# docknetwork/crypto

Measured on AMD Instinct MI355X. Metric: BLS12-381 G1 MSM/s at n=2^20 (1 GPU) and n=2^24 (8 GPU); bit-exact vs CPU, higher is better.
Workload: dtype i32 (13 signed 30-bit limbs, 381-bit modular integer; 64-bit column accumulators)

## Files before the change

crypto_amd/csrc/dock_ctx.hpp:

```cpp
#pragma once
#include <hip/hip_runtime.h>
#include <algorithm>
#include <atomic>
#include <condition_variable>
#include <cstdlib>
#include <cstring>
#include <map>
#include <mutex>
#include <vector>
#include "../../include/dock_gpu.h"
#include "host_par.hpp"

namespace dock {

extern std::atomic<uint64_t> g_dev_allocs, g_dev_alloc_ns, g_dev_alloc_bytes;
hipError_t dev_malloc(void **p, size_t bytes);

struct Buf {
    void *p = nullptr; size_t cap = 0;
    int32_t ensure(size_t bytes) {
        if (bytes <= cap) return DGPU_OK;
        if (p) { (void)hipFree(p); p = nullptr; cap = 0; }
        size_t want = bytes + bytes / 8 + 256;
        if (dev_malloc(&p, want) != hipSuccess) { (void)hipGetLastError(); if (dev_malloc(&p, bytes) != hipSuccess) { p = nullptr; return DGPU_E_OOM; } want = bytes; }
        cap = want; return DGPU_OK;
    }
    void release() { if (p) (void)hipFree(p); p = nullptr; cap = 0; }
    template <class T> T *as() { return reinterpret_cast<T *>(p); }
};

struct Handle { void *p; size_t n; int kind; int ctx; int inflight; void *aux = nullptr; int small_uses = 0; };
struct PreTable { void *tab; size_t n; int c, W; };
struct SortedScalars { void *off, *entries; size_t off_bytes, entries_bytes; size_t n, rows, boff; int c, W; };
struct FoldTab { void *tab; size_t bytes; size_t n; };
struct ShardSet { std::vector<uint64_t> sub; std::vector<size_t> lo; size_t n = 0; };
struct NttDomain { void *tw_f = nullptr, *tw_i = nullptr, *pw_f = nullptr, *pw_i = nullptr, *zinv = nullptr, *pwr_f = nullptr, *pwr_i = nullptr; };

struct ProfEntry { const char *name; double ms; uint64_t calls; };

struct Shared;
extern Shared gs;
#define HIPCHK(x) do { hipError_t e_ = (x); if (e_ != hipSuccess) { dock::gs.last_hip = (int32_t)e_; (void)hipGetLastError(); return DGPU_E_HIP; } } while (0)

struct Slot {
    std::mutex mu;
    hipStream_t stream = nullptr;
    static constexpr int N_COPY_EV = 15;
    hipStream_t cstream = nullptr;
    hipStream_t xstream = nullptr;
    void *hpin = nullptr;
    static constexpr size_t HPIN_BYTES = 64 * 1024;
    void *hpin2 = nullptr; size_t hpin2_bytes = 0;
    hipEvent_t copy_ev[N_COPY_EV + 1] = {};
    unsigned ev_next = 0;
    Buf flags, in_bases, in_inf, in_scalars, prepped, digits, heavy, cnt, off, cursor, bsums, entries, bucket, bucket_inf, head, tail, head_b, tail_b, part_inf, l1, l1_inf, win, win_inf, ml_lines, ml_partial, ml_out, ml_coeffs, ml_state, dyn, hpart, hpart_inf, small_cnt;
    Buf q[16];
    std::vector<std::pair<const char *, std::pair<hipEvent_t, hipEvent_t>>> prof_pending;
    std::vector<hipEvent_t> ev_pool;
    void release_all() {
        Buf *bufs[] = {&flags, &in_bases, &in_inf, &in_scalars, &prepped, &digits, &heavy, &cnt, &off, &cursor, &bsums, &entries, &bucket, &bucket_inf, &head, &tail, &head_b, &tail_b, &part_inf, &l1, &l1_inf, &win, &win_inf, &ml_lines, &ml_partial, &ml_out, &ml_coeffs, &ml_state, &dyn, &hpart, &hpart_inf, &small_cnt};
        for (Buf *b : bufs) b->release();
        for (Buf &b : q) b.release();
        for (hipEvent_t e : ev_pool) (void)hipEventDestroy(e);
        ev_pool.clear(); prof_pending.clear();
    }
};
constexpr int N_SLOTS = 6;

constexpr int MAX_CTX = 16;
struct Ctx {
    std::atomic<bool> ready{false};
    int device = -1;
    Slot slots[N_SLOTS];
    std::atomic<unsigned> rr{0};
    std::mutex slot_mu; std::condition_variable slot_cv; uint64_t slot_next = 0, slot_serving = 0; bool slot_taken[N_SLOTS] = {};
    std::atomic<int> busy{0};
    std::atomic<int> ml_active{0};
    std::map<int, NttDomain> ntt_domains;
    std::vector<std::pair<void *, size_t>> scalar_pool;
    size_t scalar_pool_bytes = 0;
    std::vector<std::pair<void *, size_t>> fold_pool;
};
constexpr size_t SCALAR_POOL_MAX_ENTRIES = 32, SCALAR_POOL_MAX_BYTES = (size_t)4 << 30;
struct Shared {
    std::mutex mu;
    std::mutex small_mu;
    std::condition_variable cv;
    std::map<uint64_t, Handle> handles;
    uint64_t next_handle = 1;
    std::atomic<int32_t> last_hip{0};
    std::atomic<size_t> min_gpu_n{DGPU_DEFAULT_MIN_GPU_N};
    std::atomic<size_t> auto_shard_min_n{~(size_t)0};
    std::atomic<int> window_bits{0};
// ... 146 lines not shown
```

crypto_amd/csrc/dock_dev.hip:

```cpp
#include "msm_driver.hip.h"
#include "../../include/dock_gpu_dev.h"

using namespace dock;

extern "C" {

int32_t dgpu_set_window_bits(int32_t c) { if (c != 0 && (c < 7 || c > 22)) return DGPU_E_BADARG; gs.window_bits = c; return DGPU_OK; }
int32_t dgpu_set_chunk(int32_t terms) { if (terms != 0 && (terms < 16 || terms > 4096)) return DGPU_E_BADARG; gs.chunk = terms; return DGPU_OK; }
int32_t dgpu_set_many_chunk_rows(int32_t rows) { if (rows < 0 || rows > 65535) return DGPU_E_BADARG; gs.many_chunk = rows; return DGPU_OK; }
int32_t dgpu_set_msm_segments(int32_t fold, int32_t chunk_terms) { if (fold < 0 || fold > 2 || chunk_terms < 0 || chunk_terms > (1 << 20)) return DGPU_E_BADARG; gs.seg_fold = fold; gs.seg_chunk = chunk_terms; return DGPU_OK; }
int32_t dgpu_set_reduce_lanes(int32_t lanes) { if (lanes != 0 && lanes != 1 && lanes != 2 && lanes != 4) return DGPU_E_BADARG; gs.reduce_lanes = lanes; return DGPU_OK; }
int32_t dgpu_set_reduce_shift(int32_t sh) { if (sh < -1 || sh > 6) return DGPU_E_BADARG; gs.reduce_shift = sh; return DGPU_OK; }
int32_t dgpu_set_miller_pipeline(int32_t mode) {
    if (mode < 0 || (mode & ~0x3F3F3F1F)) return DGPU_E_BADARG;
    const int a = (mode >> 8) & 63, b = (mode >> 16) & 63;
    if ((a || b) && !(a > b && b > 0 && a < 62)) return DGPU_E_BADARG;
    gs.ml_mode = mode; return DGPU_OK;
}

int32_t dgpu_prof_enable(int32_t on) { gs.prof = on != 0; return DGPU_OK; }
int32_t dgpu_prof_reset(void) { std::lock_guard<std::mutex> lk(gs.mu); gs.prof_tab.clear(); gs.allocs_at_reset = g_dev_allocs.load(); gs.alloc_ns_at_reset = g_dev_alloc_ns.load(); return DGPU_OK; }
int32_t dgpu_prof_read(const char **names, double *total_ms, uint64_t *calls, int32_t cap) {
    std::lock_guard<std::mutex> lk(gs.mu);
    int32_t k = 0;
    for (auto &t : gs.prof_tab) { if (k >= cap) break; names[k] = t.name; total_ms[k] = t.ms; calls[k] = t.calls; k++; }
    if (k < cap) { names[k] = "hipMalloc"; total_ms[k] = (double)(g_dev_alloc_ns.load() - gs.alloc_ns_at_reset) * 1e-6; calls[k] = g_dev_allocs.load() - gs.allocs_at_reset; k++; }
    return k;
}

int32_t dgpu_selftest_fp_mul(const uint64_t *a, const uint64_t *b, size_t n, uint64_t *out) {
    if (!cur().ready) return DGPU_E_NODEVICE;
    SLOT_ACQUIRE(L, sl);
    HIPCHK(hipSetDevice(cur().device));
    void *da, *db, *dout;
    HIPCHK(dev_malloc(&da, n * 48 + 16)); HIPCHK(dev_malloc(&db, n * 48 + 16)); HIPCHK(dev_malloc(&dout, n * 48 + 16));
    HIPCHK(hipMemcpy(da, a, n * 48, hipMemcpyHostToDevice)); HIPCHK(hipMemcpy(db, b, n * 48, hipMemcpyHostToDevice));
    launch_selftest_fp_mul(sl.stream, (const uint32_t *)da, (const uint32_t *)db, n, (uint32_t *)dout);
    HIPCHK(hipStreamSynchronize(sl.stream));
    HIPCHK(hipMemcpy(out, dout, n * 48, hipMemcpyDeviceToHost));
    (void)hipFree(da); (void)hipFree(db); (void)hipFree(dout);
    return DGPU_OK;
}
int32_t dgpu_selftest_g1_sum(const uint64_t *pts, const uint8_t *neg, size_t n, uint64_t out[18]) {
    if (!cur().ready) return DGPU_E_NODEVICE;
// ... 28 lines not shown
```

crypto_amd/csrc/k_g1_red.hip:

```cpp
#include "msm_launch_impl.hip.h"
namespace msm {
template void launch_fixup<G1>(hipStream_t, uint32_t, uint32_t *, uint8_t *, const uint32_t *, const uint32_t *, const uint32_t *, const uint32_t *, const uint8_t *, size_t, const uint32_t *, uint32_t, const uint32_t *);
template void launch_fixup_heavy<G1>(hipStream_t, const uint32_t *, uint32_t, const uint32_t *, uint32_t, uint32_t, uint32_t *, uint8_t *, const uint32_t *, const uint32_t *, const uint8_t *, size_t, uint32_t *, uint32_t *, uint8_t *);
template void launch_merge_buckets<G1>(hipStream_t, uint32_t, uint32_t *, uint8_t *, const uint32_t *, const uint8_t *);
template void launch_reduce_l0<G1>(hipStream_t, unsigned, const uint32_t *, const uint8_t *, uint32_t, int, uint32_t *, uint8_t *);
template void launch_reduce_top<G1>(hipStream_t, unsigned, const uint32_t *, const uint8_t *, int, int, uint32_t *, uint8_t *, int);
template void launch_reduce_top_s<G1>(hipStream_t, unsigned, const uint32_t *, const uint8_t *, int, int, uint32_t *, uint8_t *, uint32_t *, uint8_t *, int);
template int launch_reduce_marginals<G1>(hipStream_t, unsigned, const uint32_t *, const uint8_t *, uint32_t, int, uint32_t *, uint8_t *, uint32_t *, uint8_t *, bool);
template size_t reduce_marginals_points<G1>(size_t);
}
```

crypto_amd/csrc/k_g2_red.hip:

```cpp
#include "msm_launch_impl.hip.h"
namespace msm {
template void launch_merge_buckets<G2>(hipStream_t, uint32_t, uint32_t *, uint8_t *, const uint32_t *, const uint8_t *);
template void launch_reduce_l0<G2>(hipStream_t, unsigned, const uint32_t *, const uint8_t *, uint32_t, int, uint32_t *, uint8_t *);
template void launch_reduce_top<G2>(hipStream_t, unsigned, const uint32_t *, const uint8_t *, int, int, uint32_t *, uint8_t *, int);
template void launch_reduce_top_s<G2>(hipStream_t, unsigned, const uint32_t *, const uint8_t *, int, int, uint32_t *, uint8_t *, uint32_t *, uint8_t *, int);
template int launch_reduce_marginals<G2>(hipStream_t, unsigned, const uint32_t *, const uint8_t *, uint32_t, int, uint32_t *, uint8_t *, uint32_t *, uint8_t *, bool);
template size_t reduce_marginals_points<G2>(size_t);
}
```

crypto_amd/csrc/msm_driver.hip.h:

```cpp
#pragma once
#include <chrono>
#include <thread>
#include "dock_ctx.hpp"
#include "bases_cache.hpp"
#include "host_field.hpp"
#include "msm_launch.hip.h"
#include "sort_launch.hip.h"
#include "qap_launch.hip.h"

namespace dock {
using namespace msm;

template <class HF>
void host_fold(const uint64_t *win_abi, const uint8_t *win_inf, int W, int c, uint64_t *out_xyz) {
    typedef hostf::HXyzz<HF> PT;
    PT acc = PT::identity();
    const size_t FWORDS = sizeof(HF) / 8;
    for (int w = W - 1; w >= 0; w--) {
        if (!acc.inf) for (int k = 0; k < c; k++) acc.dbl_in_place();
        if (!win_inf[w]) {
            PT t; t.inf = false;
            const uint64_t *src = win_abi + (size_t)w * 4 * FWORDS;
            memcpy(&t.x, src, sizeof(HF)); memcpy(&t.y, src + FWORDS, sizeof(HF)); memcpy(&t.zz, src + 2 * FWORDS, sizeof(HF)); memcpy(&t.zzz, src + 3 * FWORDS, sizeof(HF));
            acc.add_in_place(t);
// ... 386 lines not shown
    g.T = (g.Emax + g.CH - 1) / g.CH;
    g.min_chunk = C::NFP == 2 ? 32u : 16u; g.max_chunks = C::NFP == 2 ? 150000u : 300000u; g.lanes_per_chunk = C::NFP == 2 ? 2u : 1u;
    g.HEAVY_CAP = (uint32_t)(g.Emax / (16u * 16u)) + 1;
    return DGPU_OK;
}
template <class C> int32_t ws_pre(Slot &sl, const PreTable &pt, const PreGeom &g, size_t n) {
    const uint32_t NB = g.NB; const size_t T = g.T; const int PW = g.PW;
    const uint32_t P = (NB + (1u << ps_part_log(NB)) - 1) >> ps_part_log(NB);
    const size_t n1 = (size_t)P * ((n + PS_TILE - 1) / PS_TILE);
    int32_t rc;
    if ((rc = sl.flags.ensure(64))) return rc;
    if ((rc = sl.cnt.ensure((n1 + 1) * 4))) return rc;
    if ((rc = sl.cursor.ensure((n1 + 1) * 4))) return rc;
    if ((rc = sl.bsums.ensure((scan_blocks(n1) + 2) * 4))) return rc;
    if ((rc = sl.digits.ensure(g.Emax * 8))) return rc;
    if ((rc = sl.heavy.ensure(((size_t)g.HEAVY_CAP + 1) * 4))) return rc;
    if ((rc = sl.off.ensure(((size_t)NB + 1) * 4))) return rc;
    if ((rc = sl.entries.ensure(g.Emax * 4))) return rc;
    if ((rc = sl.bucket.ensure(soa_points(NB) * C::XW * 4))) return rc;
    if ((rc = sl.bucket_inf.ensure(NB))) return rc;
    if ((rc = sl.head.ensure(soa_points(T) * C::XW * 4))) return rc;
    if ((rc = sl.tail.ensure(soa_points(T) * C::XW * 4))) return rc;
    if ((rc = sl.head_b.ensure(T * 4))) return rc;
    if ((rc = sl.tail_b.ensure(T * 4))) return rc;
    if ((rc = sl.part_inf.ensure(T * 2))) return rc;
    const size_t NGw = std::max(g.NG, (size_t)(NB >> 9)), PWw = std::max((size_t)PW, (size_t)(NB >> 15));
    const size_t mpts = reduce_marginals_points<C>(NGw);
    if ((rc = sl.l1.ensure(std::max(NGw * 2, mpts) * C::XW * 4))) return rc;
    if ((rc = sl.l1_inf.ensure(std::max(NGw * 2, mpts)))) return rc;
    if ((rc = sl.win.ensure(std::max((size_t)2 * PWw, (size_t)32) * 4 * C::ABI_W * 4))) return rc;
    if ((rc = sl.win_inf.ensure(std::max((size_t)2 * PWw, (size_t)32)))) return rc;
    if ((rc = sl.dyn.ensure(msm::dyn_words(T) * 4))) return rc;
    { const size_t hslots = 2 * (T / msm::HEAVY_RANGE + 2); if ((rc = sl.hpart.ensure(hslots * C::XW * 4))) return rc; if ((rc = sl.hpart_inf.ensure(hslots))) return rc; }
    (void)pt;
    return DGPU_OK;
}
template <class C> inline size_t pre_rows_bytes(size_t n, int W) { return (size_t)W * n * C::AFF_STRIDE * 4; }
template <class C> inline size_t pre_tab_bytes(size_t n, int W) { return pre_rows_bytes<C>(n, W) + ((n + 15) & ~(size_t)15); }
template <class C> inline const uint8_t *pre_idflags(const PreTable &pt) { return (const uint8_t *)pt.tab + pre_rows_bytes<C>(pt.n, pt.W); }
inline size_t pre_off_bytes(const PreTable &pt) { return (((size_t)1 << (pt.c - 1)) + 1) * 4; }
inline size_t pre_entries_bytes(const PreTable &pt, size_t n) { return (size_t)n * pt.W * 4; }

template <class C>
int32_t pre_sort(Slot &sl, const PreTable &pt, const PreGeom &g, size_t boff, const uint32_t *d_scalars, size_t n, uint32_t *off, uint32_t *entries, uint32_t *dyn, bool reset_flag = true) {
    PsParams q;
    q.scalars = d_scalars; q.idflag = dyn ? pre_idflags<C>(pt) : nullptr ; q.n = n; q.flag_base = (uint32_t)boff;
    q.c = pt.c; q.W = pt.W; q.key_wstride = 0; q.val_base = (uint32_t)boff; q.val_wstride = (uint32_t)pt.n;
    q.part_log = ps_part_log(g.NB); q.P = (g.NB + (1u << q.part_log) - 1) >> q.part_log; q.ntiles = (uint32_t)((n + PS_TILE - 1) / PS_TILE);
    int32_t rc;
    if ((rc = ws_pre<C>(sl, pt, g, n))) return rc;
    q.bad = sl.flags.as<uint32_t>();
    const uint32_t heavy_thr = dyn ? 16u * (uint32_t)g.CH  : 0xffffffffu ;
    const uint32_t dyn_args[6] = {(uint32_t)forced_chunk(), g.min_chunk, g.max_chunks, g.lanes_per_chunk, (uint32_t)g.T, g.NB};
    StageTimer st(sl, "msm.psort");
    HIPCHK(hipMemsetAsync(sl.heavy.p, 0, 4, sl.stream));
    if (reset_flag) HIPCHK(hipMemsetAsync(sl.flags.p, 0, 4, sl.stream));
    launch_psort(sl.stream, q, g.NB, sl.cnt.as<uint32_t>(), sl.cursor.as<uint32_t>(), sl.bsums.as<uint32_t>(), sl.digits.p, off, entries,
                 heavy_thr, sl.heavy.as<uint32_t>(), g.HEAVY_CAP, dyn_args, dyn);
    return DGPU_OK;
}
template <class C>
int32_t pre_acc(Slot &sl, const PreTable &pt, const PreGeom &g, const uint32_t *off, const uint32_t *entries, bool derive_dyn, const msm::RowMap &map, size_t set) {
    const uint32_t NB = g.NB; const size_t T = g.T;
    uint32_t *const dyn = sl.dyn.as<uint32_t>();
    const uint32_t heavy_thr = 16u * (uint32_t)g.CH;
    hipStream_t s = sl.stream;
    uint32_t *const bucket = sl.bucket.as<uint32_t>() + set * soa_points(NB) * C::XW;
    uint8_t *const bucket_inf = sl.bucket_inf.as<uint8_t>() + set * (size_t)NB;
    HIPCHK(hipMemsetAsync(bucket_inf, 1, NB, s));
    if (derive_dyn) {
        HIPCHK(hipMemsetAsync(sl.heavy.p, 0, 4, s));
        launch_dyn_chunk(s, off + NB, (uint32_t)forced_chunk(), g.min_chunk, g.max_chunks, g.lanes_per_chunk, (uint32_t)T, dyn, NB);
        launch_flag_heavy(s, off, NB, dyn, sl.heavy.as<uint32_t>(), g.HEAVY_CAP);
    }
    {
        StageTimer st(sl, "msm.accumulate");
        if (derive_dyn) launch_accumulate_skip_identity<C>(s, (const uint32_t *)pt.tab, entries, off, NB, bucket, bucket_inf,
                           sl.head.as<uint32_t>(), sl.tail.as<uint32_t>(), sl.head_b.as<uint32_t>(), sl.tail_b.as<uint32_t>(), sl.part_inf.as<uint8_t>(), T, (uint32_t)g.CH, dyn, map);
        else launch_accumulate<C>(s, (const uint32_t *)pt.tab, entries, off, NB, bucket, bucket_inf,
                           sl.head.as<uint32_t>(), sl.tail.as<uint32_t>(), sl.head_b.as<uint32_t>(), sl.tail_b.as<uint32_t>(), sl.part_inf.as<uint8_t>(), T, (uint32_t)g.CH, 0xffffffffu, dyn);
    }
    {
        StageTimer st(sl, "msm.fixup");
        launch_fixup<C>(s, NB, bucket, bucket_inf, sl.head.as<uint32_t>(), sl.tail.as<uint32_t>(),
                           sl.head_b.as<uint32_t>(), sl.tail_b.as<uint32_t>(), sl.part_inf.as<uint8_t>(), T, off, heavy_thr, dyn);
        launch_fixup_heavy<C>(s, sl.heavy.as<uint32_t>(), g.HEAVY_CAP, off, (uint32_t)g.CH, NB, bucket, bucket_inf,
                           sl.head.as<uint32_t>(), sl.tail.as<uint32_t>(), sl.part_inf.as<uint8_t>(), T, dyn, sl.hpart.as<uint32_t>(), sl.hpart_inf.as<uint8_t>());
        if (set > 0) launch_merge_buckets<C>(s, NB, sl.bucket.as<uint32_t>(), sl.bucket_inf.as<uint8_t>(), bucket, bucket_inf);
    }
    return DGPU_OK;
}
template <class C, class HF>
int32_t pre_finish(Slot &sl, const PreGeom &g, bool check_flag, uint64_t *out_xyz) {
    const uint32_t NB = g.NB; const int PW = g.PW;
    hipStream_t s = sl.stream;
    uint32_t *win_a = sl.win.as<uint32_t>(), *win_s = win_a + (size_t)PW * 4 * C::ABI_W;
    uint8_t *inf_a = sl.win_inf.as<uint8_t>(), *inf_s = inf_a + PW;
    const int rl = gs.reduce_lanes.load();
    const bool marginals = (rl == 0 || rl == 2) && g.NG >= 2;
    int nm = 0;
    {
        StageTimer st(sl, "msm.reduce");
        if (marginals) nm = launch_reduce_marginals<C>(s, (unsigned)g.NG, sl.bucket.as<uint32_t>(), sl.bucket_inf.as<uint8_t>(), NB, g.mshift, sl.l1.as<uint32_t>(), sl.l1_inf.as<uint8_t>(), win_a, inf_a, rl == 0);
        else {
            launch_reduce_l0<C>(s, (unsigned)g.NG, sl.bucket.as<uint32_t>(), sl.bucket_inf.as<uint8_t>(), NB, g.mshift, sl.l1.as<uint32_t>(), sl.l1_inf.as<uint8_t>());
            launch_reduce_top_s<C>(s, (unsigned)PW, sl.l1.as<uint32_t>(), sl.l1_inf.as<uint8_t>(), g.G, 6 + g.mshift, win_a, inf_a, win_s, inf_s, gs.reduce_lanes.load() == 1 ? 1 : 4);
        }
    }
    HIPCHK(hipGetLastError());
    const size_t npts = marginals ? (size_t)nm + 1 : (size_t)2 * PW;
    std::vector<uint64_t> hwin(npts * 2 * C::ABI_W);
    std::vector<uint8_t> hinf(npts);
    const size_t wb = npts * 4 * C::ABI_W * 4, ib = (npts + 7) & ~(size_t)7;
    std::vector<uint8_t> big;
    if (wb + ib + 4 > Slot::HPIN_BYTES) big.resize(wb + ib + 4);
    uint8_t *const hp = big.empty() ? (uint8_t *)sl.hpin : big.data();
    memset(hp + wb + ib, 0, 4);
    HIPCHK(hipMemcpyAsync(hp, sl.win.p, wb, hipMemcpyDeviceToHost, s));
    HIPCHK(hipMemcpyAsync(hp + wb, sl.win_inf.p, npts, hipMemcpyDeviceToHost, s));
    if (check_flag) HIPCHK(hipMemcpyAsync(hp + wb + ib, sl.flags.p, 4, hipMemcpyDeviceToHost, s));
    auto tsync0 = std::chrono::steady_clock::now();
    HIPCHK(hipStreamSynchronize(s));
    auto tsync1 = std::chrono::steady_clock::now();
    if (gs.prof) prof_flush(sl);
    uint32_t hbad; memcpy(&hbad, hp + wb + ib, 4);
    if (hbad) return DGPU_E_BADARG;
    memcpy(hwin.data(), hp, wb); memcpy(hinf.data(), hp + wb, npts);
    if (marginals) host_fold_marginals<HF>(hwin.data(), hinf.data(), nm, g.mshift + (C::NFP == 2 ? 1 : 0), out_xyz);
    else host_fold_shared<HF>(hwin.data(), hinf.data(), hwin.data() + (size_t)PW * 2 * C::ABI_W, hinf.data() + PW, PW, g.lb, out_xyz);
    if (gs.prof) {
        auto t2 = std::chrono::steady_clock::now();
        prof_add_host("msm.host_wait", std::chrono::duration<double, std::milli>(tsync1 - tsync0).count());
        prof_add_host("msm.host_fold", std::chrono::duration<double, std::milli>(t2 - tsync1).count());
    }
    return DGPU_OK;
}
// ... 812 lines not shown
```

crypto_amd/csrc/msm_launch.hip.h:

```cpp
#pragma once
#include <hip/hip_runtime.h>
#include "msm_kernels.hip.h"
#include "many_fold.hip.h"
#include "seg_layout.hip.h"

namespace msm {

template <class C> void launch_prep_bases(hipStream_t s, const uint32_t *abi, const uint8_t *is_inf, size_t n, uint32_t *out);
template <class C> void launch_prep_bases_fp(hipStream_t s, const uint32_t *abi, const uint8_t *is_inf, size_t n, uint32_t *out);
template <class C> void launch_prep_bases_raw(hipStream_t s, const uint8_t *raw, size_t stride, size_t x_off, size_t y_off, size_t inf_off, const uint8_t *is_inf, size_t n, uint32_t *out);
template <class C> void launch_accumulate(hipStream_t s, const uint32_t *bases, const uint32_t *entries, const uint32_t *off, uint32_t NB, uint32_t *bucket, uint8_t *bucket_inf,
                                          uint32_t *head, uint32_t *tail, uint32_t *head_b, uint32_t *tail_b, uint8_t *part_inf, size_t T, uint32_t CH, uint32_t dbg_mask, const uint32_t *dyn = nullptr);
template <class C> void launch_accumulate_skip_identity(hipStream_t s, const uint32_t *bases, const uint32_t *entries, const uint32_t *off, uint32_t NB, uint32_t *bucket, uint8_t *bucket_inf,
                                          uint32_t *head, uint32_t *tail, uint32_t *head_b, uint32_t *tail_b, uint8_t *part_inf, size_t T, uint32_t CH, const uint32_t *dyn, const RowMap &map);
template <class C> void launch_fixup(hipStream_t s, uint32_t NB, uint32_t *bucket, uint8_t *bucket_inf, const uint32_t *head, const uint32_t *tail, const uint32_t *head_b,
                                     const uint32_t *tail_b, const uint8_t *part_inf, size_t T, const uint32_t *off, uint32_t heavy_thr, const uint32_t *dyn = nullptr);
template <class C> void launch_fixup_heavy(hipStream_t s, const uint32_t *heavy, uint32_t heavy_cap, const uint32_t *off, uint32_t CH, uint32_t NB, uint32_t *bucket, uint8_t *bucket_inf,
                                           const uint32_t *head, const uint32_t *tail, const uint8_t *part_inf, size_t T, uint32_t *dyn, uint32_t *hpart, uint8_t *hpart_inf);
template <class C> void launch_merge_buckets(hipStream_t s, uint32_t NB, uint32_t *dst, uint8_t *dst_inf, const uint32_t *src, const uint8_t *src_inf);
template <class C> void launch_reduce_l0(hipStream_t s, unsigned NG, const uint32_t *bucket, const uint8_t *bucket_inf, uint32_t NB, int mshift, uint32_t *l1, uint8_t *l1_inf);
template <class C> int launch_reduce_marginals(hipStream_t s, unsigned NG, const uint32_t *bucket, const uint8_t *bucket_inf, uint32_t NB, int mshift, uint32_t *cls, uint8_t *cls_inf, uint32_t *win_abi, uint8_t *win_inf, bool quad);
template <class C> size_t reduce_marginals_points(size_t NG);
template <class C> void launch_reduce_top(hipStream_t s, unsigned W, const uint32_t *l1, const uint8_t *l1_inf, int G, int gshift, uint32_t *win_abi, uint8_t *win_inf, int lanes);

constexpr int SMALL_MSM_C = 4, SMALL_MSM_W = 64, SMALL_MSM_E = 8, SMALL_MSM_LEAVES = 128, SMALL_MSM_S = 4;
constexpr size_t SMALL_MSM_MAX_N = 8192;
inline int small_per_group(size_t L, int subtables) { const int g = (int)((L + 256 * (size_t)subtables - 1) / (256 * (size_t)subtables)); return g < 2 ? 2 : g; }
template <class C> void launch_small_table(hipStream_t s, const uint32_t *bases, size_t n, uint32_t *tab, uint8_t *tab_inf);
template <class C> void launch_small_subtable(hipStream_t s, const uint32_t *bases, size_t n, uint32_t *tab, uint8_t *tab_inf);
template <class C> void launch_small_tree(hipStream_t s, const uint32_t *tab, const uint8_t *tab_inf, int subtables, const uint32_t *scalars, size_t n, uint32_t *partial, uint8_t *partial_inf,
                                          uint32_t *count, uint32_t *win_abi, uint8_t *win_inf, uint8_t *win_bad);

template <class C> void launch_many_tree(hipStream_t s, const uint32_t *tab, const uint8_t *tab_inf, const uint32_t *scalars, size_t n, size_t row_stride, size_t rows, uint32_t *partial,
                                         uint8_t *partial_inf, uint32_t *count, uint32_t *win, uint8_t *win_inf, uint32_t *bad_flag);
template <class C> void launch_many_fold(hipStream_t s, const uint32_t *win, const uint8_t *win_inf, size_t rows, uint32_t *out_xyz, uint8_t *out_inf);

template <class C> void launch_seg_tree(hipStream_t s, const uint32_t *tab, const uint8_t *tab_inf, const uint32_t *scalars, const void *desc, size_t blocks, uint32_t *partial,
                                        uint8_t *partial_inf, uint32_t *count, uint32_t *win, uint8_t *win_inf, bool abi, uint32_t *bad_flag);
template <class C> void launch_seg_fold(hipStream_t s, const uint32_t *win, const uint8_t *win_inf, size_t nseg, uint32_t *out_xyz, uint8_t *out_inf);

template <class C> void launch_pre_step(hipStream_t s, const uint32_t *prev, size_t n, int c, uint32_t *tmp, uint32_t *out);
template <class C> void launch_reduce_top_s(hipStream_t s, unsigned W, const uint32_t *l1, const uint8_t *l1_inf, int G, int gshift, uint32_t *win_abi, uint8_t *win_inf, uint32_t *win_s_abi, uint8_t *win_s_inf, int lanes);

}
```

crypto_amd/csrc/msm_launch_impl.hip.h:

```cpp
#pragma once
#include "msm_launch.hip.h"
#include "reduce_kernels.hip.h"

namespace msm {
template <class C> void launch_prep_bases(hipStream_t s, const uint32_t *abi, const uint8_t *is_inf, size_t n, uint32_t *out) {
    hipLaunchKernelGGL((k_prep_bases<typename C::MSM>), dim3((unsigned)((n + 255) / 256)), dim3(256), 0, s, abi, is_inf, n, out);
}
template <class C> void launch_prep_bases_raw(hipStream_t s, const uint8_t *raw, size_t stride, size_t x_off, size_t y_off, size_t inf_off, const uint8_t *is_inf, size_t n, uint32_t *out) {
    hipLaunchKernelGGL((k_prep_bases_raw<typename C::MSM>), dim3((unsigned)((n + 255) / 256)), dim3(256), 0, s, raw, stride, x_off, y_off, inf_off, is_inf, n, out);
}
template <class C> void launch_prep_bases_fp(hipStream_t s, const uint32_t *abi, const uint8_t *is_inf, size_t n, uint32_t *out) {
    hipLaunchKernelGGL((k_prep_bases<C>), dim3((unsigned)((n + 255) / 256)), dim3(256), 0, s, abi, is_inf, n, out);
}
template <class C> void launch_accumulate(hipStream_t s, const uint32_t *bases, const uint32_t *entries, const uint32_t *off, uint32_t NB, uint32_t *bucket, uint8_t *bucket_inf,
                                          uint32_t *head, uint32_t *tail, uint32_t *head_b, uint32_t *tail_b, uint8_t *part_inf, size_t T, uint32_t CH, uint32_t dbg_mask, const uint32_t *dyn) {
    typedef typename C::ACC A;
    hipLaunchKernelGGL((k_accumulate<A>), dim3((unsigned)((T * A::LPP + 255) / 256)), dim3(256), 0, s, bases, entries, off, NB, bucket, bucket_inf, head, tail, head_b, tail_b, part_inf, T, CH, dbg_mask, dyn, RowMap{});
}
template <class C> void launch_accumulate_skip_identity(hipStream_t s, const uint32_t *bases, const uint32_t *entries, const uint32_t *off, uint32_t NB, uint32_t *bucket, uint8_t *bucket_inf,
                                          uint32_t *head, uint32_t *tail, uint32_t *head_b, uint32_t *tail_b, uint8_t *part_inf, size_t T, uint32_t CH, const uint32_t *dyn, const RowMap &map) {
    typedef typename C::ACC A;
    hipLaunchKernelGGL((k_accumulate<A, true>), dim3((unsigned)((T * A::LPP + 255) / 256)), dim3(256), 0, s, bases, entries, off, NB, bucket, bucket_inf, head, tail, head_b, tail_b, part_inf, T, CH, 0xffffffffu, dyn, map);
}
template <class C> void launch_fixup(hipStream_t s, uint32_t NB, uint32_t *bucket, uint8_t *bucket_inf, const uint32_t *head, const uint32_t *tail, const uint32_t *head_b,
                                     const uint32_t *tail_b, const uint8_t *part_inf, size_t T, const uint32_t *off, uint32_t heavy_thr, const uint32_t *dyn) {
    if constexpr (C::NFP == 2) hipLaunchKernelGGL((k_fixup_pair<G2P>), dim3((unsigned)((2 * T + 255) / 256)), dim3(256), 0, s, NB, bucket, bucket_inf, head, tail, head_b, tail_b, part_inf, T, off, heavy_thr, dyn);
    else hipLaunchKernelGGL((k_fixup<typename C::MSM>), dim3((unsigned)((T + 255) / 256)), dim3(256), 0, s, NB, bucket, bucket_inf, head, tail, head_b, tail_b, part_inf, T, off, heavy_thr, dyn);
}
template <class C> void launch_fixup_heavy(hipStream_t s, const uint32_t *heavy, uint32_t heavy_cap, const uint32_t *off, uint32_t CH, uint32_t NB, uint32_t *bucket, uint8_t *bucket_inf,
                                           const uint32_t *head, const uint32_t *tail, const uint8_t *part_inf, size_t T, uint32_t *dyn, uint32_t *hpart, uint8_t *hpart_inf) {
    typedef typename C::ACC A;
    hipLaunchKernelGGL((k_fixup_heavy<A>), dim3(512), dim3(A::HEAVY_T), 0, s, heavy, heavy_cap, off, CH, NB, bucket, bucket_inf, head, tail, part_inf, T, dyn);
    hipLaunchKernelGGL((k_fixup_heavy_ranges<A>), dim3(64, 32), dim3(A::HEAVY_T), 0, s, off, head, tail, part_inf, (const uint32_t *)dyn, hpart, hpart_inf);
    hipLaunchKernelGGL((k_fixup_heavy_join<A>), dim3(32), dim3(A::HEAVY_T), 0, s, off, NB, bucket, bucket_inf, (const uint32_t *)dyn, (const uint32_t *)hpart, (const uint8_t *)hpart_inf);
}
template <class C> void launch_merge_buckets(hipStream_t s, uint32_t NB, uint32_t *dst, uint8_t *dst_inf, const uint32_t *src, const uint8_t *src_inf) {
    typedef typename C::ACC A;
    hipLaunchKernelGGL((k_merge_buckets<A>), dim3((unsigned)(((size_t)NB * A::LPP + 255) / 256)), dim3(256), 0, s, NB, dst, dst_inf, src, src_inf);
}
template <class C> void launch_reduce_l0(hipStream_t s, unsigned NG, const uint32_t *bucket, const uint8_t *bucket_inf, uint32_t NB, int mshift, uint32_t *l1, uint8_t *l1_inf) {
    const unsigned blocks = (NG + 3) / 4;
    if constexpr (C::NFP == 2) hipLaunchKernelGGL((k_reduce_l0_pair<G2P>), dim3(blocks), dim3(256), 0, s, bucket, bucket_inf, NB, mshift, l1, l1_inf, NG);
    else hipLaunchKernelGGL((k_reduce_l0<typename C::MSM>), dim3(blocks), dim3(256), 0, s, bucket, bucket_inf, NB, mshift, l1, l1_inf, NG);
}
template <class C> inline void red_levels(bool quad, int &PL, int &KK) { typedef RedGeom<typename C::ACC> RG; PL = quad ? 64 : RG::PL; KK = quad ? 6 : RG::K; }
template <class C> size_t reduce_marginals_points(size_t NG) {
    typedef RedGeom<typename C::ACC> RG;
    size_t best = 0;
    for (int quad = 0; quad < 2; quad++) {
        int PL, KK; red_levels<C>(quad != 0, PL, KK);
        size_t total = (size_t)(RG::K + 2) * NG, cnt = NG; int nm = RG::K;
        while (cnt > 1) { const int steps = std::min(KK, red_log2((unsigned)cnt)); const size_t chunks = std::max<size_t>(1, cnt / PL); nm += steps; total += (size_t)(nm + 2) * chunks; cnt = chunks; }
        best = std::max(best, total + 64);
    }
    return best;
}
template <class C> int launch_reduce_marginals(hipStream_t s, unsigned NG, const uint32_t *bucket, const uint8_t *bucket_inf, uint32_t NB, int mshift, uint32_t *cls, uint8_t *cls_inf, uint32_t *win_abi, uint8_t *win_inf, bool quad) {
    typedef typename C::ACC A; typedef RedGeom<A> RG;
    hipLaunchKernelGGL((k_reduce_m0<A>), dim3((NG + 3) / 4), dim3(256), 0, s, bucket, bucket_inf, NB, mshift, cls, cls_inf, NG);
    int PL, KK; red_levels<C>(quad, PL, KK);
    unsigned cnt = NG; int nm = RG::K;
    uint32_t *in = cls; uint8_t *in_inf = cls_inf;
    while (cnt > 1) {
        const int steps = std::min(KK, red_log2(cnt));
        const unsigned chunks = std::max(1u, cnt / (unsigned)PL), npairs = 1u + (unsigned)(nm + 1) / 2u, waves = npairs * chunks;
        uint32_t *out = in + (size_t)(nm + 2) * cnt * A::XW; uint8_t *out_inf = in_inf + (size_t)(nm + 2) * cnt;
        if (quad) hipLaunchKernelGGL((k_reduce_cls_quad<A>), dim3(waves), dim3(256 * A::LPP), 0, s, (const uint32_t *)in, (const uint8_t *)in_inf, cnt, nm, out, out_inf, chunks == 1 ? 1 : 0, win_abi, win_inf);
        else hipLaunchKernelGGL((k_reduce_cls<A>), dim3((waves + 3) / 4), dim3(256), 0, s, (const uint32_t *)in, (const uint8_t *)in_inf, cnt, nm, out, out_inf, chunks == 1 ? 1 : 0, win_abi, win_inf);
        nm += steps; cnt = chunks; in = out; in_inf = out_inf;
    }
    return nm;
}
template <class C> void launch_reduce_top(hipStream_t s, unsigned W, const uint32_t *l1, const uint8_t *l1_inf, int G, int gshift, uint32_t *win_abi, uint8_t *win_inf, int lanes) {
    if (lanes == 4) {
        typedef typename C::ACC A;
        hipLaunchKernelGGL((k_reduce_top_quad<A>), dim3(W), dim3(256 * A::LPP), 0, s, l1, l1_inf, G, gshift, win_abi, win_inf, (uint32_t *)nullptr, (uint8_t *)nullptr);
        return;
    }
    if constexpr (C::NFP == 2) hipLaunchKernelGGL((k_reduce_top_pair<G2P>), dim3(W), dim3(64), 0, s, l1, l1_inf, G, gshift, win_abi, win_inf, (uint32_t *)nullptr, (uint8_t *)nullptr);
    else hipLaunchKernelGGL((k_reduce_top<typename C::MSM>), dim3(W), dim3(64), 0, s, l1, l1_inf, G, gshift, win_abi, win_inf, (uint32_t *)nullptr, (uint8_t *)nullptr);
}
template <class C> void launch_reduce_top_s(hipStream_t s, unsigned W, const uint32_t *l1, const uint8_t *l1_inf, int G, int gshift, uint32_t *win_abi, uint8_t *win_inf, uint32_t *win_s_abi, uint8_t *win_s_inf, int lanes) {
    if (lanes == 4) {
        typedef typename C::ACC A;
        hipLaunchKernelGGL((k_reduce_top_quad<A>), dim3(W), dim3(256 * A::LPP), 0, s, l1, l1_inf, G, gshift, win_abi, win_inf, win_s_abi, win_s_inf);
        return;
    }
    if constexpr (C::NFP == 2) hipLaunchKernelGGL((k_reduce_top_pair<G2P>), dim3(W), dim3(64), 0, s, l1, l1_inf, G, gshift, win_abi, win_inf, win_s_abi, win_s_inf);
    else hipLaunchKernelGGL((k_reduce_top<typename C::MSM>), dim3(W), dim3(64), 0, s, l1, l1_inf, G, gshift, win_abi, win_inf, win_s_abi, win_s_inf);
}
}
```

crypto_amd/csrc/reduce_kernels.hip.h:

```cpp
#pragma once
#include "msm_kernels.hip.h"

namespace msm {

template <class C> struct RedGeom {
    static constexpr int LPP = C::LPP;
    static constexpr int PL = 64 / LPP;
    static constexpr int K = LPP == 1 ? 6 : 5;
    static constexpr int PW = (int)(sizeof(Xyzz<typename C::F>) / 4);
};
__host__ __device__ inline int red_log2(unsigned v) { int r = 0; while ((1u << (r + 1)) <= v) r++; return r; }
inline size_t reduce_m_points(size_t NG, int PL, int K) {
    size_t total = (size_t)(K + 2) * NG; size_t cnt = NG; int nm = K;
    while (cnt > 1) { const int steps = std::min(K, red_log2((unsigned)cnt)); const size_t chunks = std::max<size_t>(1, cnt / PL); nm += steps; total += (size_t)(nm + 2) * chunks; cnt = chunks; }
    return total + 64;
}

template <class C> __device__ __forceinline__ void shfl_xor_point(Xyzz<typename C::F> &o, bool &oinf, const Xyzz<typename C::F> &x, bool xinf, int d) {
    constexpr int PW_ = RedGeom<C>::PW;
    const uint32_t *w = reinterpret_cast<const uint32_t *>(&x);
    uint32_t *q = reinterpret_cast<uint32_t *>(&o);
#pragma unroll
    for (int k = 0; k < PW_; k++) q[k] = (uint32_t)__shfl_xor((int)w[k], d * C::LPP, 64);
    oinf = __shfl_xor((int)xinf, d * C::LPP, 64) != 0;
}
template <class C> __device__ __forceinline__ void tree_step(Xyzz<typename C::F> &S, bool &sinf, Xyzz<typename C::F> &A, bool &ainf, int pl, int d, bool weighted) {
    typedef typename C::F F;
    constexpr int PW_ = RedGeom<C>::PW;
    const bool hi = (pl & d) != 0;
    uint32_t *ws = reinterpret_cast<uint32_t *>(&S), *wa = reinterpret_cast<uint32_t *>(&A);
#pragma unroll
    for (int k = 0; k < PW_; k++) { const uint32_t s = ws[k], a = wa[k]; ws[k] = hi ? a : s; wa[k] = hi ? s : a; }
    { const bool s = sinf, a = ainf; sinf = hi ? a : s; ainf = hi ? s : a; }
    Xyzz<F> o; bool oinf;
// ... 163 lines not shown
        xyzz_add_rounds(S, sinf, o, oinf || !active, q4);
#pragma unroll
        for (int k = 0; k < PW_; k++) { const uint32_t a = ws[k], b = wa[k]; ws[k] = hi ? b : a; wa[k] = hi ? a : b; }
        { const bool a = sinf, b = ainf; sinf = hi ? b : a; ainf = hi ? a : b; }
    }
    const bool outS = gi == 0, outA = has1 && gi == (1 << steps) - 1;
    const bool outM = pair == 0 && gi < (1 << steps) && gi != 0 && (gi & (gi - 1)) == 0;
    const unsigned cm = 2u + (unsigned)nm + (unsigned)red_log2((unsigned)gi);
    const bool first = t % GL == 0;
    if (!final_) {
        if (q4.role == 0) {
            if (outS) { store_soa<C>(out + (size_t)c0 * chunks * C::XW, chunks, j, S); if (first) out_inf[(size_t)c0 * chunks + j] = sinf; }
            if (outA) { store_soa<C>(out + (size_t)c1 * chunks * C::XW, chunks, j, A); if (first) out_inf[(size_t)c1 * chunks + j] = ainf; }
            if (outM) { store_soa<C>(out + (size_t)cm * chunks * C::XW, chunks, j, S); if (first) out_inf[(size_t)cm * chunks + j] = sinf; }
        }
        return;
    }
    constexpr int WS = 4 * 12 * LPP;
    auto emit = [&](unsigned c, const Xyzz<F> &pt, bool inf) __attribute__((always_inline)) {
        if (c == 0) return;
        const unsigned slot = c - 1;
        if (first) win_inf[slot] = inf;
        if (inf) return;
        const Fs *f = reinterpret_cast<const Fs *>(&pt);
        Fs v;
#pragma unroll
        for (int i = 0; i < SN; i++) v.l[i] = pick4(q4.role, f[0].l[i], f[1].l[i], f[2].l[i], f[3].l[i]);
        fs_to_abi(win_abi + (size_t)slot * WS + 12 * (LPP * q4.role + h), v);
    };
    if (outS || outM) emit(outS ? c0 : cm, S, sinf);
    if (outA) emit(c1, A, ainf);
}

}
```

Baseline: 419.6.

## Fuse final bucket-reduction levels via last-block-done atomic counters

Adds a fused reduce kernel that, once the remaining count fits in the fused limit, runs the current level and then lets the last-finishing block of each output pair, detected with atomic counters, perform the final level in the same launch. This removes the extra kernel launches and the serialised tail of small reduction levels. It adds a persistent per-slot counter buffer that must stay zeroed between calls, plus threadfence and atomic overhead, and the final level then runs on only a few blocks. Reduce-lanes mode 8 keeps the old non-fused quad path.

```diff
diff --git a/crypto_amd/csrc/dock_ctx.hpp b/crypto_amd/csrc/dock_ctx.hpp
--- a/crypto_amd/csrc/dock_ctx.hpp
+++ b/crypto_amd/csrc/dock_ctx.hpp
@@ -53,12 +53,12 @@
     void *hpin2 = nullptr; size_t hpin2_bytes = 0;
     hipEvent_t copy_ev[N_COPY_EV + 1] = {};
     unsigned ev_next = 0;
-    Buf flags, in_bases, in_inf, in_scalars, prepped, digits, heavy, cnt, off, cursor, bsums, entries, bucket, bucket_inf, head, tail, head_b, tail_b, part_inf, l1, l1_inf, win, win_inf, ml_lines, ml_partial, ml_out, ml_coeffs, ml_state, dyn, hpart, hpart_inf, small_cnt;
+    Buf flags, in_bases, in_inf, in_scalars, prepped, digits, heavy, cnt, off, cursor, bsums, entries, bucket, bucket_inf, head, tail, head_b, tail_b, part_inf, l1, l1_inf, win, win_inf, ml_lines, ml_partial, ml_out, ml_coeffs, ml_state, dyn, hpart, hpart_inf, small_cnt, red_cnt;
     Buf q[16];
     std::vector<std::pair<const char *, std::pair<hipEvent_t, hipEvent_t>>> prof_pending;
     std::vector<hipEvent_t> ev_pool;
     void release_all() {
-        Buf *bufs[] = {&flags, &in_bases, &in_inf, &in_scalars, &prepped, &digits, &heavy, &cnt, &off, &cursor, &bsums, &entries, &bucket, &bucket_inf, &head, &tail, &head_b, &tail_b, &part_inf, &l1, &l1_inf, &win, &win_inf, &ml_lines, &ml_partial, &ml_out, &ml_coeffs, &ml_state, &dyn, &hpart, &hpart_inf, &small_cnt};
+        Buf *bufs[] = {&flags, &in_bases, &in_inf, &in_scalars, &prepped, &digits, &heavy, &cnt, &off, &cursor, &bsums, &entries, &bucket, &bucket_inf, &head, &tail, &head_b, &tail_b, &part_inf, &l1, &l1_inf, &win, &win_inf, &ml_lines, &ml_partial, &ml_out, &ml_coeffs, &ml_state, &dyn, &hpart, &hpart_inf, &small_cnt, &red_cnt};
         for (Buf *b : bufs) b->release();
         for (Buf &b : q) b.release();
         for (hipEvent_t e : ev_pool) (void)hipEventDestroy(e);
diff --git a/crypto_amd/csrc/dock_dev.hip b/crypto_amd/csrc/dock_dev.hip
--- a/crypto_amd/csrc/dock_dev.hip
+++ b/crypto_amd/csrc/dock_dev.hip
@@ -9,7 +9,7 @@
 int32_t dgpu_set_chunk(int32_t terms) { if (terms != 0 && (terms < 16 || terms > 4096)) return DGPU_E_BADARG; gs.chunk = terms; return DGPU_OK; }
 int32_t dgpu_set_many_chunk_rows(int32_t rows) { if (rows < 0 || rows > 65535) return DGPU_E_BADARG; gs.many_chunk = rows; return DGPU_OK; }
 int32_t dgpu_set_msm_segments(int32_t fold, int32_t chunk_terms) { if (fold < 0 || fold > 2 || chunk_terms < 0 || chunk_terms > (1 << 20)) return DGPU_E_BADARG; gs.seg_fold = fold; gs.seg_chunk = chunk_terms; return DGPU_OK; }
-int32_t dgpu_set_reduce_lanes(int32_t lanes) { if (lanes != 0 && lanes != 1 && lanes != 2 && lanes != 4) return DGPU_E_BADARG; gs.reduce_lanes = lanes; return DGPU_OK; }
+int32_t dgpu_set_reduce_lanes(int32_t lanes) { if (lanes != 0 && lanes != 1 && lanes != 2 && lanes != 4 && lanes != 8) return DGPU_E_BADARG; gs.reduce_lanes = lanes; return DGPU_OK; }
 int32_t dgpu_set_reduce_shift(int32_t sh) { if (sh < -1 || sh > 6) return DGPU_E_BADARG; gs.reduce_shift = sh; return DGPU_OK; }
 int32_t dgpu_set_miller_pipeline(int32_t mode) {
     if (mode < 0 || (mode & ~0x3F3F3F1F)) return DGPU_E_BADARG;
diff --git a/crypto_amd/csrc/k_g1_red.hip b/crypto_amd/csrc/k_g1_red.hip
--- a/crypto_amd/csrc/k_g1_red.hip
+++ b/crypto_amd/csrc/k_g1_red.hip
@@ -6,6 +6,6 @@
 template void launch_reduce_l0<G1>(hipStream_t, unsigned, const uint32_t *, const uint8_t *, uint32_t, int, uint32_t *, uint8_t *);
 template void launch_reduce_top<G1>(hipStream_t, unsigned, const uint32_t *, const uint8_t *, int, int, uint32_t *, uint8_t *, int);
 template void launch_reduce_top_s<G1>(hipStream_t, unsigned, const uint32_t *, const uint8_t *, int, int, uint32_t *, uint8_t *, uint32_t *, uint8_t *, int);
-template int launch_reduce_marginals<G1>(hipStream_t, unsigned, const uint32_t *, const uint8_t *, uint32_t, int, uint32_t *, uint8_t *, uint32_t *, uint8_t *, bool);
+template int launch_reduce_marginals<G1>(hipStream_t, unsigned, const uint32_t *, const uint8_t *, uint32_t, int, uint32_t *, uint8_t *, uint32_t *, uint8_t *, bool, uint32_t *);
 template size_t reduce_marginals_points<G1>(size_t);
 }
diff --git a/crypto_amd/csrc/k_g2_red.hip b/crypto_amd/csrc/k_g2_red.hip
--- a/crypto_amd/csrc/k_g2_red.hip
+++ b/crypto_amd/csrc/k_g2_red.hip
@@ -4,6 +4,6 @@
 template void launch_reduce_l0<G2>(hipStream_t, unsigned, const uint32_t *, const uint8_t *, uint32_t, int, uint32_t *, uint8_t *);
 template void launch_reduce_top<G2>(hipStream_t, unsigned, const uint32_t *, const uint8_t *, int, int, uint32_t *, uint8_t *, int);
 template void launch_reduce_top_s<G2>(hipStream_t, unsigned, const uint32_t *, const uint8_t *, int, int, uint32_t *, uint8_t *, uint32_t *, uint8_t *, int);
-template int launch_reduce_marginals<G2>(hipStream_t, unsigned, const uint32_t *, const uint8_t *, uint32_t, int, uint32_t *, uint8_t *, uint32_t *, uint8_t *, bool);
+template int launch_reduce_marginals<G2>(hipStream_t, unsigned, const uint32_t *, const uint8_t *, uint32_t, int, uint32_t *, uint8_t *, uint32_t *, uint8_t *, bool, uint32_t *);
 template size_t reduce_marginals_points<G2>(size_t);
 }
diff --git a/crypto_amd/csrc/msm_driver.hip.h b/crypto_amd/csrc/msm_driver.hip.h
--- a/crypto_amd/csrc/msm_driver.hip.h
+++ b/crypto_amd/csrc/msm_driver.hip.h
@@ -442,6 +442,10 @@
     if ((rc = sl.win_inf.ensure(std::max((size_t)2 * PWw, (size_t)32)))) return rc;
     if ((rc = sl.dyn.ensure(msm::dyn_words(T) * 4))) return rc;
     { const size_t hslots = 2 * (T / msm::HEAVY_RANGE + 2); if ((rc = sl.hpart.ensure(hslots * C::XW * 4))) return rc; if ((rc = sl.hpart_inf.ensure(hslots))) return rc; }
+    if (!sl.red_cnt.p) {
+        if ((rc = sl.red_cnt.ensure((size_t)msm::RED_PLAN_COUNTERS * 4))) return rc;
+        if (hipMemsetAsync(sl.red_cnt.p, 0, (size_t)msm::RED_PLAN_COUNTERS * 4, sl.stream) != hipSuccess) { (void)hipGetLastError(); sl.red_cnt.release(); return DGPU_E_HIP; }
+    }
     (void)pt;
     return DGPU_OK;
 }
@@ -507,11 +511,11 @@
     uint32_t *win_a = sl.win.as<uint32_t>(), *win_s = win_a + (size_t)PW * 4 * C::ABI_W;
     uint8_t *inf_a = sl.win_inf.as<uint8_t>(), *inf_s = inf_a + PW;
     const int rl = gs.reduce_lanes.load();
-    const bool marginals = (rl == 0 || rl == 2) && g.NG >= 2;
+    const bool marginals = (rl == 0 || rl == 2 || rl == 8) && g.NG >= 2;
     int nm = 0;
     {
         StageTimer st(sl, "msm.reduce");
-        if (marginals) nm = launch_reduce_marginals<C>(s, (unsigned)g.NG, sl.bucket.as<uint32_t>(), sl.bucket_inf.as<uint8_t>(), NB, g.mshift, sl.l1.as<uint32_t>(), sl.l1_inf.as<uint8_t>(), win_a, inf_a, rl == 0);
+        if (marginals) nm = launch_reduce_marginals<C>(s, (unsigned)g.NG, sl.bucket.as<uint32_t>(), sl.bucket_inf.as<uint8_t>(), NB, g.mshift, sl.l1.as<uint32_t>(), sl.l1_inf.as<uint8_t>(), win_a, inf_a, rl != 2, rl == 0 ? sl.red_cnt.as<uint32_t>() : nullptr);
         else {
             launch_reduce_l0<C>(s, (unsigned)g.NG, sl.bucket.as<uint32_t>(), sl.bucket_inf.as<uint8_t>(), NB, g.mshift, sl.l1.as<uint32_t>(), sl.l1_inf.as<uint8_t>());
             launch_reduce_top_s<C>(s, (unsigned)PW, sl.l1.as<uint32_t>(), sl.l1_inf.as<uint8_t>(), g.G, 6 + g.mshift, win_a, inf_a, win_s, inf_s, gs.reduce_lanes.load() == 1 ? 1 : 4);
diff --git a/crypto_amd/csrc/msm_launch.hip.h b/crypto_amd/csrc/msm_launch.hip.h
--- a/crypto_amd/csrc/msm_launch.hip.h
+++ b/crypto_amd/csrc/msm_launch.hip.h
@@ -3,6 +3,7 @@
 #include "msm_kernels.hip.h"
 #include "many_fold.hip.h"
 #include "seg_layout.hip.h"
+#include "reduce_plan.hip.h"
 
 namespace msm {
 
@@ -19,7 +20,7 @@
                                            const uint32_t *head, const uint32_t *tail, const uint8_t *part_inf, size_t T, uint32_t *dyn, uint32_t *hpart, uint8_t *hpart_inf);
 template <class C> void launch_merge_buckets(hipStream_t s, uint32_t NB, uint32_t *dst, uint8_t *dst_inf, const uint32_t *src, const uint8_t *src_inf);
 template <class C> void launch_reduce_l0(hipStream_t s, unsigned NG, const uint32_t *bucket, const uint8_t *bucket_inf, uint32_t NB, int mshift, uint32_t *l1, uint8_t *l1_inf);
-template <class C> int launch_reduce_marginals(hipStream_t s, unsigned NG, const uint32_t *bucket, const uint8_t *bucket_inf, uint32_t NB, int mshift, uint32_t *cls, uint8_t *cls_inf, uint32_t *win_abi, uint8_t *win_inf, bool quad);
+template <class C> int launch_reduce_marginals(hipStream_t s, unsigned NG, const uint32_t *bucket, const uint8_t *bucket_inf, uint32_t NB, int mshift, uint32_t *cls, uint8_t *cls_inf, uint32_t *win_abi, uint8_t *win_inf, bool quad, uint32_t *count);
 template <class C> size_t reduce_marginals_points(size_t NG);
 template <class C> void launch_reduce_top(hipStream_t s, unsigned W, const uint32_t *l1, const uint8_t *l1_inf, int G, int gshift, uint32_t *win_abi, uint8_t *win_inf, int lanes);
 
diff --git a/crypto_amd/csrc/msm_launch_impl.hip.h b/crypto_amd/csrc/msm_launch_impl.hip.h
--- a/crypto_amd/csrc/msm_launch_impl.hip.h
+++ b/crypto_amd/csrc/msm_launch_impl.hip.h
@@ -55,7 +55,7 @@
     }
     return best;
 }
-template <class C> int launch_reduce_marginals(hipStream_t s, unsigned NG, const uint32_t *bucket, const uint8_t *bucket_inf, uint32_t NB, int mshift, uint32_t *cls, uint8_t *cls_inf, uint32_t *win_abi, uint8_t *win_inf, bool quad) {
+template <class C> int launch_reduce_marginals(hipStream_t s, unsigned NG, const uint32_t *bucket, const uint8_t *bucket_inf, uint32_t NB, int mshift, uint32_t *cls, uint8_t *cls_inf, uint32_t *win_abi, uint8_t *win_inf, bool quad, uint32_t *count) {
     typedef typename C::ACC A; typedef RedGeom<A> RG;
     hipLaunchKernelGGL((k_reduce_m0<A>), dim3((NG + 3) / 4), dim3(256), 0, s, bucket, bucket_inf, NB, mshift, cls, cls_inf, NG);
     int PL, KK; red_levels<C>(quad, PL, KK);
@@ -65,6 +65,11 @@
         const int steps = std::min(KK, red_log2(cnt));
         const unsigned chunks = std::max(1u, cnt / (unsigned)PL), npairs = 1u + (unsigned)(nm + 1) / 2u, waves = npairs * chunks;
         uint32_t *out = in + (size_t)(nm + 2) * cnt * A::XW; uint8_t *out_inf = in_inf + (size_t)(nm + 2) * cnt;
+        if (quad && count && cnt <= RED_PLAN_MAX_FUSED) {
+            hipLaunchKernelGGL((k_reduce_cls_fused<A>), dim3(waves), dim3(256 * A::LPP), 0, s, (const uint32_t *)in, (const uint8_t *)in_inf, cnt, nm, out, out_inf, count, win_abi, win_inf);
+            while (cnt > 1) { nm += std::min(KK, red_log2(cnt)); cnt = std::max(1u, cnt / (unsigned)PL); }
+            break;
+        }
         if (quad) hipLaunchKernelGGL((k_reduce_cls_quad<A>), dim3(waves), dim3(256 * A::LPP), 0, s, (const uint32_t *)in, (const uint8_t *)in_inf, cnt, nm, out, out_inf, chunks == 1 ? 1 : 0, win_abi, win_inf);
         else hipLaunchKernelGGL((k_reduce_cls<A>), dim3((waves + 3) / 4), dim3(256), 0, s, (const uint32_t *)in, (const uint8_t *)in_inf, cnt, nm, out, out_inf, chunks == 1 ? 1 : 0, win_abi, win_inf);
         nm += steps; cnt = chunks; in = out; in_inf = out_inf;
diff --git a/crypto_amd/csrc/reduce_kernels.hip.h b/crypto_amd/csrc/reduce_kernels.hip.h
--- a/crypto_amd/csrc/reduce_kernels.hip.h
+++ b/crypto_amd/csrc/reduce_kernels.hip.h
@@ -1,5 +1,6 @@
 #pragma once
 #include "msm_kernels.hip.h"
+#include "reduce_plan.hip.h"
 
 namespace msm {
 
@@ -229,4 +230,110 @@
     if (outA) emit(c1, A, ainf);
 }
 
-}
+template <class C>
+__global__ void __launch_bounds__(256 * C::LPP) k_reduce_cls_fused(const uint32_t *in, const uint8_t *in_inf, unsigned cnt, int nm, uint32_t *out, uint8_t *out_inf,
+                                                                   uint32_t *__restrict__ count, uint32_t *__restrict__ win_abi, uint8_t *__restrict__ win_inf) {
+    typedef typename C::F F;
+    constexpr int LPP = C::LPP, GL = 4 * LPP, PW_ = 4 * SN, PLQ = 64;
+    __shared__ uint32_t xs[64 * LPP * PW_];
+    __shared__ uint8_t fl[64];
+    __shared__ uint32_t won_s;
+    const int t = (int)threadIdx.x, gi = t / GL, h = t % LPP;
+    const QuadLanes<LPP> q4;
+    const bool first = t % GL == 0;
+    const unsigned chunks = cnt / PLQ ? cnt / PLQ : 1u;
+    const uint32_t *src = in; const uint8_t *src_inf = in_inf;
+    unsigned n = cnt; int m = nm;
+    unsigned pair = blockIdx.x / chunks, j = blockIdx.x % chunks, li = (unsigned)gi;
+    bool valid = true, final_ = chunks == 1;
+    unsigned won = 0, pass = 0, npass = 1;
+    Xyzz<F> S, A;
+    uint32_t *ws = reinterpret_cast<uint32_t *>(&S), *wa = reinterpret_cast<uint32_t *>(&A);
+#pragma unroll 1
+    for (;;) {
+        const int steps = red_log2(n) < 6 ? red_log2(n) : 6;
+        const unsigned c0 = pair == 0 ? 0u : 2u * pair, c1 = c0 + 1;
+        const bool has1 = c1 < 2u + (unsigned)m;
+        const unsigned idx = j * PLQ + li;
+        bool sinf = true, ainf = true;
+        fzero(S.x); fzero(S.y); fzero(S.zz); fzero(S.zzz); A = S;
+        if (valid && idx < n) {
+            sinf = src_inf[(size_t)c0 * n + idx] != 0;
+            if (!sinf) load_soa<C>(S, src + (size_t)c0 * n * C::XW, n, idx);
+            if (has1) { ainf = src_inf[(size_t)c1 * n + idx] != 0; if (!ainf) load_soa<C>(A, src + (size_t)c1 * n * C::XW, n, idx); }
+        }
+#pragma unroll 1
+        for (int s = 0; s < steps; s++) {
+            const int d = 1 << s;
+            const bool hi = (li & (unsigned)d) != 0;
+#pragma unroll
+            for (int k = 0; k < PW_; k++) { const uint32_t a = ws[k], b = wa[k]; ws[k] = hi ? b : a; wa[k] = hi ? a : b; }
+            { const bool a = sinf, b = ainf; sinf = hi ? b : a; ainf = hi ? a : b; }
+            __syncthreads();
+            { uint32_t *dst = xs + ((gi * 4 + q4.role) * LPP + h) * SN;
+#pragma unroll
+              for (int k = 0; k < SN; k++) dst[k] = pick4(q4.role, wa[k], wa[SN + k], wa[2 * SN + k], wa[3 * SN + k]);
+              if (first) fl[gi] = ainf; }
+            __syncthreads();
+            Xyzz<F> o; bool oinf;
+            { const int sg = gi ^ d;
+              uint32_t *ov = reinterpret_cast<uint32_t *>(&o);
+#pragma unroll
+              for (int c = 0; c < 4; c++) {
+                  const uint32_t *sv = xs + ((sg * 4 + c) * LPP + h) * SN;
+#pragma unroll
+                  for (int k = 0; k < SN; k++) ov[c * SN + k] = sv[k];
+              }
+              oinf = fl[sg] != 0; }
+            const unsigned low = li & (unsigned)(d - 1);
+            const bool active = hi ? (low == (unsigned)(d - 1)) : (low == 0 || (pair == 0 && (low & (low - 1)) == 0));
+            xyzz_add_rounds(S, sinf, o, oinf || !active, q4);
+#pragma unroll
+            for (int k = 0; k < PW_; k++) { const uint32_t a = ws[k], b = wa[k]; ws[k] = hi ? b : a; wa[k] = hi ? a : b; }
+            { const bool a = sinf, b = ainf; sinf = hi ? b : a; ainf = hi ? a : b; }
+        }
+        const bool outS = valid && li == 0, outA = valid && has1 && li == (1u << steps) - 1;
+        const bool outM = valid && pair == 0 && li < (1u << steps) && li != 0 && (li & (li - 1)) == 0;
+        const unsigned cm = 2u + (unsigned)m + (unsigned)red_log2(li);
+        if (final_) {
+            constexpr int WS = 4 * 12 * LPP;
+            auto emit = [&](unsigned c, const Xyzz<F> &pt, bool inf) __attribute__((always_inline)) {
+                if (c == 0) return;
+                const unsigned slot = c - 1;
+                if (first) win_inf[slot] = inf;
+                if (inf) return;
+                const Fs *f = reinterpret_cast<const Fs *>(&pt);
+                Fs v;
+#pragma unroll
+                for (int i = 0; i < SN; i++) v.l[i] = pick4(q4.role, f[0].l[i], f[1].l[i], f[2].l[i], f[3].l[i]);
+                fs_to_abi(win_abi + (size_t)slot * WS + 12 * (LPP * q4.role + h), v);
+            };
+            if (outS || outM) emit(outS ? c0 : cm, S, sinf);
+            if (outA) emit(c1, A, ainf);
+            if (++pass >= npass) return;
+        } else {
+            if (q4.role == 0) {
+                if (outS) { store_soa<C>(out + (size_t)c0 * chunks * C::XW, chunks, j, S); if (first) out_inf[(size_t)c0 * chunks + j] = sinf; }
+                if (outA) { store_soa<C>(out + (size_t)c1 * chunks * C::XW, chunks, j, A); if (first) out_inf[(size_t)c1 * chunks + j] = ainf; }
+                if (outM) { store_soa<C>(out + (size_t)cm * chunks * C::XW, chunks, j, S); if (first) out_inf[(size_t)cm * chunks + j] = sinf; }
+            }
+            __threadfence();
+            __syncthreads();
+            if (t == 0) {
+                const unsigned feeds = red_plan_feeds(pair, m, m + steps);
+                unsigned mask = 0;
+                for (unsigned q = 0; q < (unsigned)RED_PLAN_COUNTERS; q++)
+                    if (((feeds >> q) & 1u) && atomicAdd(&count[q], 1u) + 1u == red_plan_target(q, m, chunks)) { mask |= 1u << q; count[q] = 0; }
+                won_s = mask;
+            }
+            __syncthreads();
+            won = won_s;
+            if (won == 0) return;
+            __threadfence();
+            src = out; src_inf = out_inf; n = chunks; m += steps; j = 0; final_ = true; pass = 0; npass = red_plan_passes(won, n);
+        }
+        pair = red_plan_pass_pair(won, n, pass, (unsigned)gi); valid = pair < 32u; li = (unsigned)gi % n;
+    }
+}
+
+}
diff --git a/crypto_amd/csrc/reduce_plan.hip.h b/crypto_amd/csrc/reduce_plan.hip.h
--- /dev/null
+++ b/crypto_amd/csrc/reduce_plan.hip.h
@@ -0,0 +1,38 @@
+#pragma once
+#if defined(__HIPCC__)
+#define RPFD __host__ __device__ inline
+#else
+#define RPFD inline
+#endif
+
+namespace msm {
+
+constexpr int RED_PLAN_COUNTERS = 32;
+constexpr unsigned RED_PLAN_MAX_FUSED = 4096;
+
+RPFD unsigned red_plan_npairs(int nm) { return 1u + (unsigned)(nm + 1) / 2u; }
+RPFD unsigned red_plan_first_new(int nm) { return (unsigned)(nm + 2) / 2u; }
+RPFD bool red_plan_mixed(unsigned q, int nm) { return (nm & 1) != 0 && q == (unsigned)(nm + 1) / 2u; }
+RPFD unsigned red_plan_target(unsigned q, int nm, unsigned chunks) { return red_plan_mixed(q, nm) ? 2u * chunks : chunks; }
+RPFD unsigned red_plan_feeds(unsigned pair, int nm, int nmB) {
+    if (pair != 0) return 1u << pair;
+    unsigned m = 1u;
+    for (unsigned q = red_plan_first_new(nm); q < red_plan_npairs(nmB); q++) m |= 1u << q;
+    return m;
+}
+RPFD unsigned red_plan_kth(unsigned mask, unsigned k) {
+    for (unsigned q = 0; q < 32u; q++) if ((mask >> q) & 1u) { if (k == 0) return q; k--; }
+    return 32u;
+}
+RPFD unsigned red_plan_pass_pair(unsigned mask, unsigned chunks, unsigned pass, unsigned gi) {
+    const unsigned per = 64u / chunks, k = pass * per + gi / chunks;
+    unsigned n = 0; for (unsigned q = 0; q < 32u; q++) n += (mask >> q) & 1u;
+    return k < n ? red_plan_kth(mask, k) : 32u;
+}
+RPFD unsigned red_plan_passes(unsigned mask, unsigned chunks) {
+    unsigned n = 0; for (unsigned q = 0; q < 32u; q++) n += (mask >> q) & 1u;
+    const unsigned per = 64u / chunks;
+    return (n + per - 1) / per;
+}
+
+}
```

Result: no change. 421.3 (median of 4 runs) (+0.4%).
